# Prisma-Multimodal/ViT-Prisma

Hardware: NVIDIA H100
Metric: SAE training tokens/sec (TopK SAE, d_model=768, dict=768x32, k=32) (higher is better)
Workload: dtype fp32

## Files before the change

vit-prisma_b200/csrc/sae.cu:

```cuda
#include "common.cuh"
#include "tc_common.cuh"
#include "sae_optim.cuh"

template <int CHUNKS>
__global__ void __launch_bounds__(256) k_sae_prep(const float* __restrict__ x, const float* __restrict__ b_dec, float* __restrict__ sae_in,
                                                  float* __restrict__ sae_in_lo, __half* __restrict__ sae_in16, float* __restrict__ mu_out,
                                                  float* __restrict__ std_out, int rows, int d, int norm_mode, float eps) {
  pb_pdl();
  const int lane = threadIdx.x & 31;
  const int row = blockIdx.x * (blockDim.x >> 5) + (threadIdx.x >> 5);
  if (row >= rows) return;
  const int nvec = d >> 2;
  const float* xr = x + (int64_t)row * d;
  float v[CHUNKS][4];
  float sum = 0.f;
#pragma unroll
  for (int i = 0; i < CHUNKS; ++i) {
    const int c4 = i * 32 + lane;
    if (c4 < nvec) { ld4(xr + 4 * c4, v[i]); sum += (v[i][0] + v[i][1]) + (v[i][2] + v[i][3]); }
    else v[i][0] = v[i][1] = v[i][2] = v[i][3] = 0.f;
  }
  float mu = 0.f, inv = 1.f, sd = 1.f;
  if (norm_mode == 1) {
    mu = warp_sum(sum) / (float)d;
// ... 277 lines not shown
      if (p < F) c.x = cnt[p];
      if (p + 1 < F) c.y = cnt[p + 1];
      if (p + 2 < F) c.z = cnt[p + 2];
    }
    v[i] = (int)c.x; v[i + 1] = (int)c.y; v[i + 2] = (int)c.z; v[i + 3] = (int)c.w;
  }
  int run = 0;
#pragma unroll
  for (int i = 0; i < PER; ++i) { const int x = v[i]; v[i] = run; run += x; }
  int x = run;
#pragma unroll
  for (int o = 1; o < 32; o <<= 1) {
    const int y = __shfl_up_sync(0xffffffffu, x, o);
    if (lane >= o) x += y;
  }
  if (lane == 31) wtot[warp] = x;
  __syncthreads();
  if (warp == 0) {
    int w = wtot[lane];
#pragma unroll
    for (int o = 1; o < 32; o <<= 1) {
      const int y = __shfl_up_sync(0xffffffffu, w, o);
      if (lane >= o) w += y;
    }
    wtot[lane] = w;
  }
  __syncthreads();
  const int excl = (warp ? wtot[warp - 1] : 0) + x - run;
#pragma unroll
  for (int i = 0; i < PER; i += 4) {
    const int p = base + i;
    const int4 o4 = make_int4(excl + v[i], excl + v[i + 1], excl + v[i + 2], excl + v[i + 3]);
    if (p + 3 < F) {
      *reinterpret_cast<int4*>(off + p) = o4;
      *reinterpret_cast<int4*>(cursor + p) = o4;
    } else {
      const int o[4] = {o4.x, o4.y, o4.z, o4.w};
      for (int j = 0; j < 4; ++j)
        if (p + j < F) { off[p + j] = o[j]; cursor[p + j] = o[j]; }
    }
  }
  if (t == 1023) off[F] = wtot[31];
}
__global__ void __launch_bounds__(256) k_csc_fill(const int* __restrict__ idx, int* __restrict__ cursor, int* __restrict__ entries, int64_t n) {
  pb_pdl();
  for (int64_t e = (int64_t)blockIdx.x * blockDim.x + threadIdx.x; e < n; e += (int64_t)gridDim.x * blockDim.x) {
    const int f = idx[e];
    const int pos = atomicAdd(cursor + f, 1);
    entries[pos] = (int)e;
  }
}

constexpr int SAE_LONG_LIST = 32;
constexpr int SAE_LONG_CHUNK = 32;
struct SaeWorkHeader { int n_chunks, n_long, next_f, pad; };
constexpr int SAE_CLAIM = 4;

template <int CHUNKS>
__global__ void __launch_bounds__(256) k_sae_grads(const int* __restrict__ off, int* __restrict__ entries, const float* __restrict__ val,
                                                   const float* __restrict__ dval, const float* __restrict__ g, const float* __restrict__ sae_in,
                                                   const float* __restrict__ W_encT, float* __restrict__ gW_dec, float* __restrict__ gW_encT,
                                                   float* __restrict__ gb_enc, float* __restrict__ gbdec2, float* __restrict__ fired,
                                                   SaeScalars* __restrict__ sc, int F, int d, int k, SaeWorkHeader* __restrict__ work,
                                                   int* __restrict__ work_feats, int* __restrict__ work_chunks) {
  pb_pdl();
  extern __shared__ __align__(16) float sm_bd[];
  const int lane = threadIdx.x & 31, warp = threadIdx.x >> 5, nw = blockDim.x >> 5;
  const int nvec = d >> 2;
  for (int c = threadIdx.x; c < d; c += blockDim.x) sm_bd[c] = 0.f;
  __syncthreads();
  float nsq = 0.f;
  float bd[CHUNKS][4];
#pragma unroll
  for (int i = 0; i < CHUNKS; ++i) bd[i][0] = bd[i][1] = bd[i][2] = bd[i][3] = 0.f;
  for (;;) {
    int fbase = 0;
    if (lane == 0) fbase = atomicAdd(&work->next_f, SAE_CLAIM);
    fbase = __shfl_sync(0xffffffffu, fbase, 0);
    if (fbase >= F) break;
   for (int f = fbase; f < min(F, fbase + SAE_CLAIM); ++f) {
    const int e0 = off[f], e1 = off[f + 1];
    const int len = e1 - e0;
    if (len > SAE_LONG_LIST) {
#pragma unroll
      for (int i = 0; i < CHUNKS; ++i) {
        const int c4 = i * 32 + lane;
        if (c4 < nvec) {
          const float z4[4] = {0.f, 0.f, 0.f, 0.f};
          st4(gW_dec + (int64_t)f * d + 4 * c4, z4);
          st4(gW_encT + (int64_t)f * d + 4 * c4, z4);
        }
      }
      const int nchunks = (len + SAE_LONG_CHUNK - 1) / SAE_LONG_CHUNK;
      int base = 0, lslot = 0;
      if (lane == 0) {
        gb_enc[f] = 0.f;
        fired[f] = 0.f;
        base = atomicAdd(&work->n_chunks, nchunks);
        lslot = atomicAdd(&work->n_long, 1);
        work_feats[lslot] = f;
      }
      base = __shfl_sync(0xffffffffu, base, 0);
      for (int c = lane; c < nchunks; c += 32) {
        work_chunks[2 * (base + c)] = f;
        work_chunks[2 * (base + c) + 1] = e0 + c * SAE_LONG_CHUNK;
      }
      continue;
    }
    int my_b = 0;
    float my_a = 0.f, my_dp = 0.f;
    {
      const int mine = lane < len ? entries[e0 + lane] : 0x7fffffff;
      int rank = 0;
#pragma unroll
      for (int j = 0; j < 32; ++j) rank += __shfl_sync(0xffffffffu, mine, j) < mine ? 1 : 0;
      int src = 0;
#pragma unroll
      for (int j = 0; j < 32; ++j) src = (__shfl_sync(0xffffffffu, rank, j) == lane && j < len) ? j : src;
      const int sorted = __shfl_sync(0xffffffffu, mine, src);
      if (lane < len) {
        my_b = sorted / k;
        my_a = fmaxf(val[sorted], 0.f);
        my_dp = dval[sorted];
      }
    }
    float ad[CHUNKS][4], ae[CHUNKS][4];
#pragma unroll
    for (int i = 0; i < CHUNKS; ++i) ad[i][0] = ad[i][1] = ad[i][2] = ad[i][3] = ae[i][0] = ae[i][1] = ae[i][2] = ae[i][3] = 0.f;
    float gbe = 0.f;
    const float npos = (float)__popc(__ballot_sync(0xffffffffu, my_a > 0.f));
#pragma unroll 2
    for (int j = 0; j < len; ++j) {
      const float a = __shfl_sync(0xffffffffu, my_a, j), dp = __shfl_sync(0xffffffffu, my_dp, j);
      const int b = __shfl_sync(0xffffffffu, my_b, j);
      gbe += dp;
      const float* gr = g + (int64_t)b * d;
      const float* sr = sae_in + (int64_t)b * d;
#pragma unroll
      for (int i = 0; i < CHUNKS; ++i) {
        const int c4 = i * 32 + lane;
        if (c4 < nvec) {
          float gv[4], sv[4];
          ld4(gr + 4 * c4, gv);
          ld4(sr + 4 * c4, sv);
#pragma unroll
          for (int q = 0; q < 4; ++q) { ad[i][q] = fmaf(a, gv[q], ad[i][q]); ae[i][q] = fmaf(dp, sv[q], ae[i][q]); }
        }
      }
    }
#pragma unroll
    for (int i = 0; i < CHUNKS; ++i) {
      const int c4 = i * 32 + lane;
      if (c4 < nvec) {
        st4(gW_dec + (int64_t)f * d + 4 * c4, ad[i]);
        st4(gW_encT + (int64_t)f * d + 4 * c4, ae[i]);
#pragma unroll
        for (int q = 0; q < 4; ++q) nsq += ad[i][q] * ad[i][q] + ae[i][q] * ae[i][q];
        if (gbe != 0.f) {
          float w[4];
          ld4(W_encT + (int64_t)f * d + 4 * c4, w);
#pragma unroll
          for (int q = 0; q < 4; ++q) bd[i][q] = fmaf(gbe, w[q], bd[i][q]);
        }
      }
    }
    if (lane == 0) {
      gb_enc[f] = gbe;
      fired[f] = npos;
      nsq += gbe * gbe;
    }
   }
  }
#pragma unroll
  for (int i = 0; i < CHUNKS; ++i) {
    const int c4 = i * 32 + lane;
    if (c4 < nvec) {
#pragma unroll
      for (int q = 0; q < 4; ++q)
        if (bd[i][q] != 0.f) atomicAdd(&sm_bd[4 * c4 + q], bd[i][q]);
    }
  }
  nsq = warp_sum(nsq);
  __shared__ float red[8];
  if (lane == 0) red[warp] = nsq;
  __syncthreads();
  if (threadIdx.x == 0) {
    float a = 0.f;
    for (int i = 0; i < nw; ++i) a += red[i];
    atomicAdd(&sc->gnorm_sq, a);
  }
  for (int c = threadIdx.x; c < d; c += blockDim.x)
    if (sm_bd[c] != 0.f) atomicAdd(gbdec2 + c, sm_bd[c]);
}

template <int CHUNKS>
__global__ void __launch_bounds__(256) k_sae_grads_long(const int* __restrict__ off, const int* __restrict__ entries, const float* __restrict__ val,
                                                        const float* __restrict__ dval, const float* __restrict__ g,
                                                        const float* __restrict__ sae_in, const float* __restrict__ W_encT,
                                                        float* __restrict__ gW_dec, float* __restrict__ gW_encT, float* __restrict__ gb_enc,
                                                        float* __restrict__ gbdec2, float* __restrict__ fired, int d, int k,
                                                        const SaeWorkHeader* __restrict__ work, const int* __restrict__ work_chunks) {
  pb_pdl();
  extern __shared__ __align__(16) float sm_bd[];
  const int lane = threadIdx.x & 31, warp = threadIdx.x >> 5, nw = blockDim.x >> 5;
  const int nvec = d >> 2;
  const int n_items = work->n_chunks;
  if (n_items == 0) return;
  for (int c = threadIdx.x; c < d; c += blockDim.x) sm_bd[c] = 0.f;
  __syncthreads();
  float bd[CHUNKS][4];
#pragma unroll
  for (int i = 0; i < CHUNKS; ++i) bd[i][0] = bd[i][1] = bd[i][2] = bd[i][3] = 0.f;
  for (int item = blockIdx.x * nw + warp; item < n_items; item += gridDim.x * nw) {
    const int f = work_chunks[2 * item], p0 = work_chunks[2 * item + 1];
    const int p1 = min(off[f + 1], p0 + SAE_LONG_CHUNK);
    float ad[CHUNKS][4], ae[CHUNKS][4];
#pragma unroll
    for (int i = 0; i < CHUNKS; ++i) ad[i][0] = ad[i][1] = ad[i][2] = ad[i][3] = ae[i][0] = ae[i][1] = ae[i][2] = ae[i][3] = 0.f;
    const int n = p1 - p0;
    int my_b = 0;
    float my_a = 0.f, my_dp = 0.f;
    if (lane < n) {
      const int e = entries[p0 + lane];
      my_b = e / k;
      my_a = fmaxf(val[e], 0.f);
      my_dp = dval[e];
    }
    float gbe = 0.f;
    const float npos = (float)__popc(__ballot_sync(0xffffffffu, my_a > 0.f));
#pragma unroll 2
    for (int j = 0; j < n; ++j) {
      const float a = __shfl_sync(0xffffffffu, my_a, j), dp = __shfl_sync(0xffffffffu, my_dp, j);
      const int b = __shfl_sync(0xffffffffu, my_b, j);
      gbe += dp;
      const float* gr = g + (int64_t)b * d;
      const float* sr = sae_in + (int64_t)b * d;
#pragma unroll
      for (int i = 0; i < CHUNKS; ++i) {
        const int c4 = i * 32 + lane;
        if (c4 < nvec) {
          float gv[4], sv[4];
          ld4(gr + 4 * c4, gv);
          ld4(sr + 4 * c4, sv);
#pragma unroll
          for (int q = 0; q < 4; ++q) { ad[i][q] = fmaf(a, gv[q], ad[i][q]); ae[i][q] = fmaf(dp, sv[q], ae[i][q]); }
        }
      }
    }
#pragma unroll
    for (int i = 0; i < CHUNKS; ++i) {
      const int c4 = i * 32 + lane;
      if (c4 < nvec) {
        atomicAdd(reinterpret_cast<float4*>(gW_dec + (int64_t)f * d + 4 * c4), make_float4(ad[i][0], ad[i][1], ad[i][2], ad[i][3]));
        atomicAdd(reinterpret_cast<float4*>(gW_encT + (int64_t)f * d + 4 * c4), make_float4(ae[i][0], ae[i][1], ae[i][2], ae[i][3]));
        if (gbe != 0.f) {
          float w[4];
          ld4(W_encT + (int64_t)f * d + 4 * c4, w);
#pragma unroll
          for (int q = 0; q < 4; ++q) bd[i][q] = fmaf(gbe, w[q], bd[i][q]);
        }
      }
    }
    if (lane == 0) {
      atomicAdd(gb_enc + f, gbe);
      atomicAdd(fired + f, npos);
    }
  }
#pragma unroll
  for (int i = 0; i < CHUNKS; ++i) {
    const int c4 = i * 32 + lane;
    if (c4 < nvec) {
#pragma unroll
      for (int q = 0; q < 4; ++q)
        if (bd[i][q] != 0.f) atomicAdd(&sm_bd[4 * c4 + q], bd[i][q]);
    }
  }
  __syncthreads();
  for (int c = threadIdx.x; c < d; c += blockDim.x)
    if (sm_bd[c] != 0.f) atomicAdd(gbdec2 + c, sm_bd[c]);
}

__global__ void __launch_bounds__(256) k_sae_norm_long(const float* __restrict__ gW_dec, const float* __restrict__ gW_encT,
                                                       const float* __restrict__ gb_enc, SaeScalars* __restrict__ sc, int d,
                                                       const SaeWorkHeader* work, const int* __restrict__ work_feats) {
  pb_pdl();
  const int lane = threadIdx.x & 31, warp = threadIdx.x >> 5, nw = blockDim.x >> 5;
  const int n = *reinterpret_cast<const volatile int*>(&work->n_long);
  float nsq = 0.f;
  for (int li = blockIdx.x * nw + warp; li < n; li += gridDim.x * nw) {
    const int f = work_feats[li];
    for (int c = lane; c < d; c += 32) {
      const float a = gW_dec[(int64_t)f * d + c], b = gW_encT[(int64_t)f * d + c];
      nsq += a * a + b * b;
    }
    if (lane == 0) nsq += gb_enc[f] * gb_enc[f];
  }
  nsq = warp_sum(nsq);
  if (lane == 0 && nsq != 0.f) atomicAdd(&sc->gnorm_sq, nsq);
}

__global__ void k_sae_gbdec(const float* __restrict__ gcol, const float* __restrict__ gbdec2, float* __restrict__ gb_dec, int d) {
  const int c = blockIdx.x * blockDim.x + threadIdx.x;
  if (c < d) gb_dec[c] = gcol[c] - gbdec2[c];
}

__global__ void __launch_bounds__(256) k_sae_finalize(const float* __restrict__ gcol, const float* __restrict__ gbdec2, float* __restrict__ gb_dec,
                                                      SaeScalars* __restrict__ sc, int d, float max_norm, float inv_elems, float inv_rows) {
  pb_pdl();
  __shared__ float red[8];
  float s = 0.f;
  for (int c = threadIdx.x; c < d; c += blockDim.x) {
    const float v = gcol[c] - gbdec2[c];
    gb_dec[c] = v;
    s += v * v;
  }
  s = warp_sum(s);
  if ((threadIdx.x & 31) == 0) red[threadIdx.x >> 5] = s;
  __syncthreads();
  if (threadIdx.x == 0) {
    float t = sc->gnorm_sq;
    for (int i = 0; i < 8; ++i) t += red[i];
    sae_publish_scalars(sc, t, max_norm, inv_elems, inv_rows);
  }
}

struct AdamRowsOut {
  float *W_dec, *W_encT, *W_encT_lo;
  __half* W_encT16;
  int64_t base;
  __device__ __forceinline__ void dec(int c4, const float (&w)[4]) const { st4(W_dec + base + 4 * c4, w); }
  __device__ __forceinline__ void enc(int c4, const float (&p)[4], const float (&lo)[4], uint2 p16) const {
    st4(W_encT + base + 4 * c4, p);
    if (W_encT_lo) st4(W_encT_lo + base + 4 * c4, lo);
    if (W_encT16) *reinterpret_cast<uint2*>(W_encT16 + base + 4 * c4) = p16;
  }
};

__device__ __forceinline__ void atomic_max_norm(float* out, float best_sq) {
  if (best_sq > 0.f) atomicMax(reinterpret_cast<unsigned int*>(out), __float_as_uint(sqrtf(best_sq)));
}

template <int CHUNKS>
__global__ void __launch_bounds__(256) k_sae_adam_rows(float* __restrict__ W_dec, float* __restrict__ W_encT, float* __restrict__ W_encT_lo,
                                                       __half* __restrict__ W_encT16, float* __restrict__ enc16_lo_max,
                                                       float* __restrict__ b_enc, const float* __restrict__ gW_dec,
                                                       const float* __restrict__ gW_encT, const float* __restrict__ gb_enc,
                                                       float* __restrict__ m_dec, float* __restrict__ v_dec, float* __restrict__ m_enc,
                                                       float* __restrict__ v_enc, float* __restrict__ m_be, float* __restrict__ v_be,
                                                       const float* __restrict__ fired, float* __restrict__ since_fired,
                                                       float* __restrict__ act_freq, const SaeScalars* __restrict__ sc, AdamHyper h,
                                                       int F, int d, int renorm, float* __restrict__ enc_norm_max) {
// ... 299 lines not shown
}

extern "C" int pb_sae_step_reset(const PbSaeStep* s, int32_t* fb_count, pb_stream_t stream) {
  PB_CHECK_ARG(s && s->feat_count && s->scalars && s->gcol && s->gbdec2, "pb_sae_step_reset: missing pointers");
  PB_CHECK_ARG(!s->work || s->work_bytes >= (int64_t)sizeof(SaeWorkHeader), "pb_sae_step_reset: work buffer too small");
  const int n = s->F > s->d ? s->F : s->d;
  int grid = (n + 255) / 256;
  if (grid > pb_sm_count() * 2) grid = pb_sm_count() * 2;
  if (grid * 256 < s->d) grid = (s->d + 255) / 256;
  PB_LAUNCH_PDL(k_sae_step_reset, grid, 256, 0, (cudaStream_t)stream, s->feat_count, s->F, (float*)s->scalars, s->gcol, s->gbdec2, s->d, (int*)s->work, fb_count);
  return PB_OK;
}

extern "C" int pb_sae_decode(const PbSaeStep* s, pb_stream_t stream) {
  PB_CHECK_ARG(s && s->x && s->xsum && s->idx && s->val && s->W_dec && s->b_dec && s->scalars, "pb_sae_decode: missing pointers");
  PB_CHECK_ARG(!s->training || (s->g && s->dval), "pb_sae_decode: training needs g and dval buffers");
  if (s->rows == 0) return PB_OK;
  cudaStream_t st = (cudaStream_t)stream;
  const int d = s->d, ch = chunks_for(d);
  PB_DISPATCH_CHUNKS(ch, PB_LAUNCH_PDL(k_sae_decode<C_>, (s->rows + 7) / 8, 256, 0, st,
      s->x, s->xsum, s->mu, s->sd, s->idx, s->val, s->W_dec, s->b_dec, s->sae_out, s->g, s->dval, (SaeScalars*)s->scalars, s->rows, d, s->k,
      s->norm_mode, s->training, 1.f / (float)(s->global_rows > 0 ? s->global_rows : s->rows)));
  if (!s->training) {
    k_sae_fwd_scalars<<<1, 1, 0, st>>>((SaeScalars*)s->scalars, 1.f / ((float)s->rows * (float)d), 1.f / (float)s->rows);
    PB_LAUNCH_CHECK();
  }
  return PB_OK;
}

extern "C" int pb_sae_backward(const PbSaeStep* s, pb_stream_t stream) {
  PB_CHECK_ARG(s && s->idx && s->val && s->dval && s->g && s->sae_in && s->W_encT && s->feat_count && s->csc_off && s->csc_cursor &&
               s->csc_entries && s->gW_dec && s->gW_encT && s->gb_enc && s->gb_dec && s->gcol && s->gbdec2 && s->fired && s->scalars,
               "pb_sae_backward: missing pointers");
  if (s->rows == 0) return PB_OK;
  cudaStream_t st = (cudaStream_t)stream;
  const int d = s->d, F = s->F, ch = chunks_for(d);
  {
    const int per = ((F + 1023) / 1024 + 3) / 4 * 4;
    PB_CHECK_ARG(per <= 128, "pb_sae_backward: d_sae=%d too large for the offset scan (max 131072)", F);
    if (per <= 8) PB_LAUNCH_PDL(k_scan_counts<8>, 1, 1024, 0, st, s->feat_count, s->csc_off, s->csc_cursor, F);
    else if (per <= 24) PB_LAUNCH_PDL(k_scan_counts<24>, 1, 1024, 0, st, s->feat_count, s->csc_off, s->csc_cursor, F);
    else if (per <= 48) PB_LAUNCH_PDL(k_scan_counts<48>, 1, 1024, 0, st, s->feat_count, s->csc_off, s->csc_cursor, F);
    else if (per <= 64) PB_LAUNCH_PDL(k_scan_counts<64>, 1, 1024, 0, st, s->feat_count, s->csc_off, s->csc_cursor, F);
    else PB_LAUNCH_PDL(k_scan_counts<128>, 1, 1024, 0, st, s->feat_count, s->csc_off, s->csc_cursor, F);
  }
  const int64_t n = (int64_t)s->rows * s->k;
  PB_LAUNCH_PDL(k_csc_fill, pb_sm_count() * 4, 256, 0, st, (const int*)s->idx, s->csc_cursor, s->csc_entries, n);
  if (!s->pre_zeroed) {
    PB_CUDA(cudaMemsetAsync(s->gcol, 0, sizeof(float) * d, st));
    PB_CUDA(cudaMemsetAsync(s->gbdec2, 0, sizeof(float) * d, st));
  }
  const int rpc = 8;
  PB_LAUNCH_PDL(k_colsum, (s->rows + rpc - 1) / rpc, 256, 0, st, (const float*)s->g, s->gcol, s->rows, d, rpc);
  const int64_t cap = n / SAE_LONG_CHUNK + F + 1;
  const int64_t need = (int64_t)sizeof(SaeWorkHeader) + 4 * (int64_t)F + 8 * cap;
  PB_CHECK_ARG(s->work && s->work_bytes >= need, "pb_sae_backward: work buffer too small (%lld < %lld bytes)", (long long)s->work_bytes,
               (long long)need);
  SaeWorkHeader* wh = (SaeWorkHeader*)s->work;
  int* work_feats = (int*)(wh + 1);
  int* work_chunks = work_feats + F;
  if (!s->pre_zeroed) PB_CUDA(cudaMemsetAsync(wh, 0, sizeof(SaeWorkHeader), st));
  const int grid = persistent_grid(8, F);
  PB_DISPATCH_CHUNKS(ch, PB_LAUNCH_PDL(k_sae_grads<C_>, grid, 256, sizeof(float) * d, st, s->csc_off, s->csc_entries, s->val, s->dval, s->g, s->sae_in,
                                       s->W_encT, s->gW_dec, s->gW_encT, s->gb_enc, s->gbdec2, s->fired, (SaeScalars*)s->scalars, F, d, s->k, wh,
                                       work_feats, work_chunks));
  PB_DISPATCH_CHUNKS(ch, PB_LAUNCH_PDL(k_sae_grads_long<C_>, pb_sm_count() * 4, 256, sizeof(float) * d, st, s->csc_off, s->csc_entries, s->val, s->dval,
                                       s->g, s->sae_in, s->W_encT, s->gW_dec, s->gW_encT, s->gb_enc, s->gbdec2, s->fired, d, s->k, wh, work_chunks));
  if (!s->dist) {
    PB_LAUNCH_PDL(k_sae_norm_long, pb_sm_count(), 256, 0, st, s->gW_dec, s->gW_encT, s->gb_enc, (SaeScalars*)s->scalars, d, wh, work_feats);
  }
  if (s->dist) {
    k_sae_gbdec<<<(d + 255) / 256, 256, 0, st>>>(s->gcol, s->gbdec2, s->gb_dec, d);
    PB_LAUNCH_CHECK();
    return PB_OK;
  }
  PB_LAUNCH_PDL(k_sae_finalize, 1, 256, 0, st, s->gcol, s->gbdec2, s->gb_dec, (SaeScalars*)s->scalars, d, s->max_grad_norm,
                1.f / ((float)s->rows * (float)d), 1.f / (float)s->rows);
  return PB_OK;
}

extern "C" int pb_sae_adam(const PbSaeStep* s, pb_stream_t stream) {
  PB_CHECK_ARG(s && s->W_dec && s->W_encT && s->b_enc && s->b_dec && s->gW_dec && s->gW_encT && s->gb_enc && s->gb_dec && s->m_dec &&
               s->v_dec && s->m_enc && s->v_enc && s->m_be && s->v_be && s->m_bd && s->v_bd && s->fired && s->scalars,
               "pb_sae_adam: missing pointers");
  PB_CHECK_ARG(s->step >= 1, "pb_sae_adam: step counter starts at 1");
  cudaStream_t st = (cudaStream_t)stream;
  const int d = s->d, F = s->F, ch = chunks_for(d);
  const AdamHyper h = adam_hyper(s->lr, s->beta1, s->beta2, s->adam_eps, s->step);
  const int grid = persistent_grid(8, F);
  PB_CHECK_ARG(!s->W_encT16 == !s->enc16_lo_max, "pb_sae_adam: W_encT16 and enc16_lo_max go together");
  PB_CHECK_ARG(!s->W_encT16 || (d % 8 == 0 && ((uintptr_t)s->W_encT16 & 15) == 0), "pb_sae_adam: the fp16 copy of W_encT needs d %% 8 == 0");
  __half* const W16 = (__half*)s->W_encT16;
  if (s->enc_norm_max) PB_CUDA(cudaMemsetAsync(s->enc_norm_max, 0, 2 * sizeof(float), st));
  if (s->enc16_lo_max) PB_CUDA(cudaMemsetAsync(s->enc16_lo_max, 0, sizeof(float), st));
  if (!s->W_encT_lo && d >= 64) {
    const size_t stage = (size_t)8 * d * 4;
    int S = (int)((200 * 1024) / stage);
    if (S > 12) S = 12;
    if (S >= 3) {
      const size_t smem = 256 + (size_t)S * stage;
      int g2 = pb_sm_count();
      if (g2 > F) g2 = F;
      PB_DISPATCH_CHUNKS(ch, {
        auto kern = k_sae_adam_bulk<C_>;
        PB_CUDA(cudaFuncSetAttribute(kern, cudaFuncAttributeMaxDynamicSharedMemorySize, (int)smem));
        PB_LAUNCH_PDL(kern, g2, 32 * (1 + S), smem, st, s->W_dec, s->W_encT, s->b_enc, s->gW_dec, s->gW_encT, s->gb_enc, s->m_dec, s->v_dec,
                      s->m_enc, s->v_enc, s->m_be, s->v_be, s->fired, s->since_fired, s->act_freq, (const SaeScalars*)s->scalars, h, F, d,
                      s->renorm_decoder, s->enc_norm_max, S, s->b_dec, s->gb_dec, s->m_bd, s->v_bd, W16, s->enc16_lo_max);
      });
      return PB_OK;
    }
  }
  PB_DISPATCH_CHUNKS(ch, (k_sae_adam_rows<C_><<<grid, 256, 0, st>>>(s->W_dec, s->W_encT, s->W_encT_lo, W16, s->enc16_lo_max, s->b_enc, s->gW_dec,
                                                                     s->gW_encT, s->gb_enc,
                                                                     s->m_dec, s->v_dec, s->m_enc, s->v_enc, s->m_be, s->v_be, s->fired,
                                                                     s->since_fired, s->act_freq, (const SaeScalars*)s->scalars, h,
                                                                     F, d, s->renorm_decoder, s->enc_norm_max)));
  PB_LAUNCH_CHECK();
  k_sae_adam_vec<<<(d + 255) / 256, 256, 0, st>>>(s->b_dec, s->gb_dec, s->m_bd, s->v_bd, (const SaeScalars*)s->scalars, h, d);
  PB_LAUNCH_CHECK();
  return PB_OK;
}
// ... 63 lines not shown
```

vit-prisma_b200/vit_prisma/b200/sae_engine.py:

```python
from __future__ import annotations

import ctypes as C
from typing import Optional

import torch

from . import _lib as L
from .ops import _need_cuda, _stream, cast as _cast


def ops_cast_f32(x: torch.Tensor) -> torch.Tensor:
    return _cast(x.contiguous(), torch.float32)

vp, i32, i64, f32 = C.c_void_p, C.c_int32, C.c_int64, C.c_float


class PbSaeStep(C.Structure):
    _fields_ = (
        [(n, i32) for n in ("rows", "d", "F", "k", "norm_mode", "training", "step", "renorm_decoder")]
        + [(n, f32) for n in ("lr", "beta1", "beta2", "adam_eps", "max_grad_norm")]
        + [(n, vp) for n in (
            "x", "W_encT", "W_encT_lo", "W_dec", "b_enc", "b_dec",
            "sae_in", "mu", "sd", "xsum", "idx", "val", "feat_count", "sae_out", "g", "dval",
            "csc_off", "csc_cursor", "csc_entries", "gW_dec", "gW_encT", "gb_enc", "gb_dec", "gcol", "gbdec2",
# ... 116 lines not shown
            encoder = "fused" if (fused_ok and gemm_impl == L.GEMM_AUTO) else "dense"
        if encoder == "fused" and not fused_ok:
            raise L.PrismaB200Error(f"fused encoder->TopK needs d_in % 4 == 0, d_sae % 128 == 0, k <= 48 (d={self.d} F={self.F} k={self.k})")
        self.cand_operands = ("f16" if f16_ok else "tf32") if encoder == "fused" else None
        import os
        self.encoder, self.c_keep = encoder, int(os.environ.get("PRISMA_SAE_C_KEEP", c_keep))
        self.m_cand = int(os.environ.get("PRISMA_SAE_M_CAND", 0)) or (int(m_cand) if m_cand else self.k + 8)
        self.enc_norm_max = z(2)
        self.fb_count = z(2, dt=torch.int32)
        self.W_encT_lo = torch.empty_like(W_encT) if encoder == "dense" else None
        f16 = self.cand_operands == "f16"
        self.W_encT16 = torch.empty(self.F, self.d, dtype=torch.float16, device=dev) if f16 else None
        self.enc16_lo_max = z(1) if f16 else None
        self.refresh_lo()
        self.m_dec, self.v_dec, self.m_enc, self.v_enc = z(self.F, self.d), z(self.F, self.d), z(self.F, self.d), z(self.F, self.d)
        self.m_be, self.v_be, self.m_bd, self.v_bd = z(self.F), z(self.F), z(self.d), z(self.d)
        self.gW_dec, self.gW_encT = torch.empty(self.F, self.d, device=dev), torch.empty(self.F, self.d, device=dev)
        self.gb_enc, self.gb_dec = z(self.F), z(self.d)
        self.gcol, self.gbdec2, self.xsum = z(self.d), z(self.d), z(self.d)
        self.feat_count, self.fired = z(self.F), z(self.F)
        self.csc_off, self.csc_cursor = z(self.F + 1, dt=torch.int32), z(self.F, dt=torch.int32)
        self.scalars = z(8)
        self.step_count = 0
        self._rows = -1

    def refresh_lo(self) -> None:
        if self.W_encT_lo is not None:
            from . import ops
            self.W_encT_lo.copy_(ops.split_tf32(self.W_encT))
        L.check(L.get_lib().pb_rownorm_max(self.W_encT.data_ptr(), self.F, self.d, self.enc_norm_max.data_ptr(), _stream()), "pb_rownorm_max")
        if self.W_encT16 is not None:
            L.check(L.get_lib().pb_f16_copy(self.W_encT.data_ptr(), self.F, self.d, self.W_encT16.data_ptr(), self.enc16_lo_max.data_ptr(),
                                            _stream()), "pb_f16_copy")

    def _ensure_rows(self, rows: int) -> None:
        if rows == self._rows:
            return
        dev, d, F, k = self.W_dec.device, self.d, self.F, self.k
        e = lambda *s, dt=torch.float32: torch.empty(*s, dtype=dt, device=dev)
        self.sae_in, self.g, self.sae_out = e(rows, d), e(rows, d), e(rows, d)
        self.mu, self.sd = e(rows), e(rows)
        if self.encoder == "fused":
            cb, sb = i64(0), i64(0)
            L.check(L.get_lib().pb_sae_fused_workspace(rows, F, self.c_keep, C.byref(cb), C.byref(sb)), "pb_sae_fused_workspace")
            self.cand = e(max(cb.value // 4, 4), dt=torch.int32)
            self.fb_rows = e(max(rows, 1), dt=torch.int32)
            self.fb_scratch = e(min(64, max(sb.value // (4 * F), 1)) * F)
            self.sae_in_lo = self.hidden_pre = None
            self.sae_in16 = e(rows, d, dt=torch.float16) if self.cand_operands == "f16" else None
        else:
            self.sae_in_lo, self.hidden_pre = e(rows, d), e(rows, F)
        self.idx, self.val, self.dval = e(rows, k, dt=torch.int32), e(rows, k), e(rows, k)
        self.csc_entries = e(rows * k, dt=torch.int32)
        self.work = e(8 + 4 * F + 8 * (rows * k // 32 + F + 1) + 64, dt=torch.uint8)
        nseg = (F + TOPK_SEG - 1) // TOPK_SEG
        self.topk_scratch = e(max(rows * nseg * k * 8, 16), dt=torch.uint8) if F > TOPK_SEG else None
        self._rows = rows

    def _desc(self, x: torch.Tensor, training: bool, lr: float = 0.0, since_fired=None, act_freq=None, want_out=True) -> PbSaeStep:
        s = PbSaeStep()
        s.rows, s.d, s.F, s.k = x.shape[0], self.d, self.F, self.k
        s.norm_mode, s.training, s.step, s.renorm_decoder = self.norm_mode, int(training), max(self.step_count, 1), 1
        s.lr, s.beta1, s.beta2, s.adam_eps, s.max_grad_norm = lr, self.betas[0], self.betas[1], self.adam_eps, self.max_grad_norm
        p = lambda t: None if t is None else t.data_ptr()
        s.x = p(x)
        s.W_encT, s.W_encT_lo, s.W_dec, s.b_enc, s.b_dec = p(self.W_encT), p(self.W_encT_lo), p(self.W_dec), p(self.b_enc), p(self.b_dec)
        s.sae_in, s.mu, s.sd, s.xsum = p(self.sae_in), p(self.mu), p(self.sd), p(self.xsum)
        s.idx, s.val, s.feat_count = p(self.idx), p(self.val), p(self.feat_count)
        s.sae_out, s.g, s.dval = (p(self.sae_out) if want_out else None), p(self.g), p(self.dval)
        s.csc_off, s.csc_cursor, s.csc_entries = p(self.csc_off), p(self.csc_cursor), p(self.csc_entries)
        s.gW_dec, s.gW_encT, s.gb_enc, s.gb_dec = p(self.gW_dec), p(self.gW_encT), p(self.gb_enc), p(self.gb_dec)
        s.gcol, s.gbdec2, s.fired, s.scalars = p(self.gcol), p(self.gbdec2), p(self.fired), p(self.scalars)
        s.m_dec, s.v_dec, s.m_enc, s.v_enc = p(self.m_dec), p(self.v_dec), p(self.m_enc), p(self.v_enc)
        s.m_be, s.v_be, s.m_bd, s.v_bd = p(self.m_be), p(self.v_be), p(self.m_bd), p(self.v_bd)
        s.since_fired, s.act_freq = p(since_fired), p(act_freq)
        s.work, s.work_bytes = p(self.work), self.work.numel()
        s.enc_norm_max = p(self.enc_norm_max)
        s.W_encT16, s.enc16_lo_max = p(self.W_encT16), p(self.enc16_lo_max)
        return s

    def _enc_desc(self, rows: int, phases: int = 0) -> PbSaeEncode:
        e = PbSaeEncode()
        e.rows, e.d, e.F, e.k, e.c_keep, e.m_cand, e.phases, e.err_coef = rows, self.d, self.F, self.k, self.c_keep, self.m_cand, phases, 0.0
        e.sae_in, e.W_encT, e.b_enc, e.enc_norm_max = self.sae_in.data_ptr(), self.W_encT.data_ptr(), self.b_enc.data_ptr(), self.enc_norm_max.data_ptr()
        e.cand, e.cand_bytes = self.cand.data_ptr(), self.cand.numel() * 4
        e.idx, e.val, e.feat_count = self.idx.data_ptr(), self.val.data_ptr(), self.feat_count.data_ptr()
        e.fb_count, e.fb_rows = self.fb_count.data_ptr(), self.fb_rows.data_ptr()
        e.fb_scratch, e.fb_scratch_bytes = self.fb_scratch.data_ptr(), self.fb_scratch.numel() * 4
        if self.cand_operands == "f16":
            e.sae_in16, e.W_encT16, e.enc16_lo_max = self.sae_in16.data_ptr(), self.W_encT16.data_ptr(), self.enc16_lo_max.data_ptr()
        return e

    def _encoder_gemm(self, rows: int) -> None:
        lib, st = L.get_lib(), _stream()
        use_tc = self.gemm_impl != L.GEMM_SIMT
        g = L.PbGemm()
        g.M, g.N, g.K, g.dtype, g.impl = rows, self.F, self.d, L.PB_F32, self.gemm_impl
        g.A, g.lda, g.B, g.ldb = self.sae_in.data_ptr(), self.d, self.W_encT.data_ptr(), self.d
        if use_tc:
            g.A_lo, g.B_lo = self.sae_in_lo.data_ptr(), self.W_encT_lo.data_ptr()
        g.bias, g.out0, g.ld0 = self.b_enc.data_ptr(), self.hidden_pre.data_ptr(), self.F
        L.check(lib.pb_gemm(C.byref(g), st), "pb_gemm(encoder)")

    def encode_topk(self, x: torch.Tensor, pre_zeroed: bool = False) -> None:
        lib, st = L.get_lib(), _stream()
        rows = x.shape[0]
        self._ensure_rows(rows)
# ... 54 lines not shown
        return int(self.fb_count[0].item()) if self.encoder == "fused" else 0

    def rescored_per_row(self, rows: int) -> float:
        fb, tot = self.fb_count.tolist()
        return tot / max(rows - fb, 1)

    def _optimizer_stages(self, s: PbSaeStep, x: torch.Tensor, lr: float, since_fired, act_freq):
        lib, st = L.get_lib(), _stream()
        kernel = "k_sae_adam_rows" if self.W_encT_lo is not None or self.d < 64 else "k_sae_adam_bulk"
        f16_copy = 2 * self.d * self.F if self.W_encT16 is not None else 0
        return [("adam (clip + decoder-parallel-gradient removal + Adam + row renorm)", lambda: L.check(lib.pb_sae_adam(C.byref(s), st)),
                 dict(bytes=60 * self.d * self.F + f16_copy, ncu=kernel))]

    def _clip_and_adam(self, x: torch.Tensor, lr: float, since_fired, act_freq, grads, extra) -> None:
        lib, st = L.get_lib(), _stream()
        self.scalars[1:2].zero_()
        acc = self.scalars[1:].data_ptr()
        for t in grads:
            L.check(lib.pb_sumsq(t.data_ptr(), t.numel(), acc, st), "pb_sumsq")
        L.check(lib.pb_sae_clip_finish(self.scalars.data_ptr(), self.max_grad_norm, x.shape[0], self.d, st), "pb_sae_clip_finish")
        s = self._desc(x, training=True, lr=lr, since_fired=since_fired, act_freq=act_freq, want_out=False)
        L.check(lib.pb_sae_adam(C.byref(s), st), "pb_sae_adam")
        for p, g, m, v in extra:
            L.check(lib.pb_adam_vec(p.data_ptr(), g.data_ptr(), m.data_ptr(), v.data_ptr(), p.numel(), self.scalars.data_ptr(), lr, self.betas[0],
                                    self.betas[1], self.adam_eps, self.step_count, st), "pb_adam_vec")

    @torch.no_grad()
    def time_stages(self, x: torch.Tensor, lr: float, since_fired=None, act_freq=None, reps: int = 5) -> dict:
        lib, st = L.get_lib(), _stream()
        x = ops_cast_f32(x)
        rows = x.shape[0]
        out = {}

        def timed(name, fn, **info):
            torch.cuda.synchronize()
            a, b = torch.cuda.Event(enable_timing=True), torch.cuda.Event(enable_timing=True)
            a.record()
            for _ in range(reps):
                fn()
            b.record()
            torch.cuda.synchronize()
            out[name] = dict(ms=a.elapsed_time(b) / reps, **info)

        for name, fn, info in self._encode_stages(x):
            timed(name, fn, **info)
        self.encode_topk(x)
        self.scalars.zero_()
        self.step_count += 1
        s = self._desc(x, training=True, lr=float(lr), since_fired=since_fired, act_freq=act_freq, want_out=False)
        self._prepare_timed_step(s, x)
        timed("decode (sparse decode + loss + d_hidden)", lambda: L.check(lib.pb_sae_decode(C.byref(s), st)),
              bytes=(12 * rows * self.d + 8 * rows * self.k), ncu=r"k_sae_decode")
        timed("backward (csc build + per-feature gradients + norm)", lambda: (self.scalars.zero_(), L.check(lib.pb_sae_backward(C.byref(s), st))),
              bytes=8 * self.d * self.F, ncu=r"k_sae_grads<")
        for name, fn, info in self._optimizer_stages(s, x, float(lr), since_fired, act_freq):
            timed(name, fn, **info)
        return out

    def _prepare_timed_step(self, s: PbSaeStep, x: torch.Tensor) -> None:
        pass

    def _encode_stages(self, x: torch.Tensor):
        rows = x.shape[0]
        if self.encoder == "fused":
            lib, st = L.get_lib(), _stream()
            self.encode_topk(x)
            flops = 2.0 * rows * self.d * self.F
            nkeys = (self.F // 128) * self.c_keep
            op, es = ("fp16", 2) if self.cand_operands == "f16" else ("tf32", 4)
            return [(f"encode + topk, fused (prep + {op} candidate GEMM + select / exact re-score + exact path)", lambda: self.encode_topk(x),
                     dict(flops=flops, passes=1)),
                    (f"candidate GEMM alone (one {op} pass, top-c-per-segment epilogue)",
                     lambda: L.check(lib.pb_sae_encode_topk_fused(C.byref(self._enc_desc(rows, 1)), st)),
                     dict(flops=flops, passes=1, bytes=es * self.d * self.F + es * rows * self.d + 4 * rows * nkeys, ncu=r"k_enc_cand")),
                    ("select + exact re-score alone", lambda: L.check(lib.pb_sae_encode_topk_fused(C.byref(self._enc_desc(rows, 2)), st)),
                     dict(bytes=4 * rows * nkeys + 4 * rows * self.d + 8 * rows * self.k, ncu=r"k_cand_select"))]
        return [("encode + topk (prep + encoder GEMM 3xTF32 + exact topk)", lambda: self.encode_topk(x),
                 dict(flops=2.0 * rows * self.d * self.F, passes=3, ncu=r"k_gemm_tc<float")),
                ("encoder GEMM alone (hidden_pre = sae_in @ W_enc + b_enc)", lambda: self._encoder_gemm(rows),
                 dict(flops=2.0 * rows * self.d * self.F, passes=3, bytes=8 * self.d * self.F + 8 * rows * self.d + 4 * rows * self.F))]

    def dense_feature_acts(self) -> torch.Tensor:
        rows = self.idx.shape[0]
        dense = torch.empty(rows, self.F, device=self.W_dec.device)
        L.check(L.get_lib().pb_sae_scatter_acts(self.idx.data_ptr(), self.val.data_ptr(), dense.data_ptr(), rows, self.k, self.F, 1,
                                                _stream()), "pb_sae_scatter_acts")
        return dense

    def scalars_dict(self) -> dict:
        vals = self.scalars.tolist()
        return dict(zip(SCALAR_NAMES, vals))

    def algorithmic_bytes(self, rows: int) -> int:
        return 80 * self.d * self.F + 8 * rows * self.d
```

Baseline: 3.038 million.

## Replace chunked long-feature gradient path with token-sorted pack and column-sliced smem kernel

Features with many firing tokens are no longer split into 32-entry chunks that accumulate into the weight gradients with float4 atomics. A new pack kernel sorts each long feature's entries by token using a bitmap and prefix sums, and writes packed token, activation and d-value arrays. It also computes gb_enc, fired and the bias norm term. A column-sliced kernel then stages 8-column slices of g and sae_in for all rows in shared memory and lets each warp compute the full gradient for one feature over that slice, writing the result directly and folding in the norm, which removes the separate norm kernel. This trades global gather traffic and atomics for a large shared-memory footprint, row chunking with binary searches when rows exceed the smem capacity, and an added cap on rows from the bitmap.

```diff
diff --git a/vit-prisma_b200/csrc/sae.cu b/vit-prisma_b200/csrc/sae.cu
--- a/vit-prisma_b200/csrc/sae.cu
+++ b/vit-prisma_b200/csrc/sae.cu
@@ -353,9 +353,12 @@
 }
 
 constexpr int SAE_LONG_LIST = 32;
-constexpr int SAE_LONG_CHUNK = 32;
-struct SaeWorkHeader { int n_chunks, n_long, next_f, pad; };
+struct SaeWorkHeader { int next_f, n_long, pad[2]; };
 constexpr int SAE_CLAIM = 4;
+constexpr int SAE_SLICE = 8;
+constexpr int SAE_SLICE_THREADS = 1024;
+constexpr int SAE_SLICE_PARTS = 2;
+constexpr int SAE_SLICE_SMEM = 192 * 1024;
 
 template <int CHUNKS>
 __global__ void __launch_bounds__(256) k_sae_grads(const int* __restrict__ off, int* __restrict__ entries, const float* __restrict__ val,
@@ -363,7 +366,7 @@
                                                    const float* __restrict__ W_encT, float* __restrict__ gW_dec, float* __restrict__ gW_encT,
                                                    float* __restrict__ gb_enc, float* __restrict__ gbdec2, float* __restrict__ fired,
                                                    SaeScalars* __restrict__ sc, int F, int d, int k, SaeWorkHeader* __restrict__ work,
-                                                   int* __restrict__ work_feats, int* __restrict__ work_chunks) {
+                                                   int* __restrict__ work_feats) {
   pb_pdl();
   extern __shared__ __align__(16) float sm_bd[];
   const int lane = threadIdx.x & 31, warp = threadIdx.x >> 5, nw = blockDim.x >> 5;
@@ -383,29 +386,7 @@
     const int e0 = off[f], e1 = off[f + 1];
     const int len = e1 - e0;
     if (len > SAE_LONG_LIST) {
-#pragma unroll
-      for (int i = 0; i < CHUNKS; ++i) {
-        const int c4 = i * 32 + lane;
-        if (c4 < nvec) {
-          const float z4[4] = {0.f, 0.f, 0.f, 0.f};
-          st4(gW_dec + (int64_t)f * d + 4 * c4, z4);
-          st4(gW_encT + (int64_t)f * d + 4 * c4, z4);
-        }
-      }
-      const int nchunks = (len + SAE_LONG_CHUNK - 1) / SAE_LONG_CHUNK;
-      int base = 0, lslot = 0;
-      if (lane == 0) {
-        gb_enc[f] = 0.f;
-        fired[f] = 0.f;
-        base = atomicAdd(&work->n_chunks, nchunks);
-        lslot = atomicAdd(&work->n_long, 1);
-        work_feats[lslot] = f;
-      }
-      base = __shfl_sync(0xffffffffu, base, 0);
-      for (int c = lane; c < nchunks; c += 32) {
-        work_chunks[2 * (base + c)] = f;
-        work_chunks[2 * (base + c) + 1] = e0 + c * SAE_LONG_CHUNK;
-      }
+      if (lane == 0) work_feats[atomicAdd(&work->n_long, 1)] = f;
       continue;
     }
     int my_b = 0;
@@ -494,110 +475,184 @@
     if (sm_bd[c] != 0.f) atomicAdd(gbdec2 + c, sm_bd[c]);
 }
 
-template <int CHUNKS>
-__global__ void __launch_bounds__(256) k_sae_grads_long(const int* __restrict__ off, const int* __restrict__ entries, const float* __restrict__ val,
-                                                        const float* __restrict__ dval, const float* __restrict__ g,
-                                                        const float* __restrict__ sae_in, const float* __restrict__ W_encT,
-                                                        float* __restrict__ gW_dec, float* __restrict__ gW_encT, float* __restrict__ gb_enc,
-                                                        float* __restrict__ gbdec2, float* __restrict__ fired, int d, int k,
-                                                        const SaeWorkHeader* __restrict__ work, const int* __restrict__ work_chunks) {
+__global__ void __launch_bounds__(256) k_sae_pack_long(const int* __restrict__ off, const int* __restrict__ entries, const float* __restrict__ val,
+                                                       const float* __restrict__ dval, int* __restrict__ ptok, float* __restrict__ pa,
+                                                       float* __restrict__ pd, float* __restrict__ gb_enc, float* __restrict__ fired,
+                                                       SaeScalars* __restrict__ sc, int rows, int k, const SaeWorkHeader* work,
+                                                       const int* __restrict__ work_feats) {
   pb_pdl();
-  extern __shared__ __align__(16) float sm_bd[];
-  const int lane = threadIdx.x & 31, warp = threadIdx.x >> 5, nw = blockDim.x >> 5;
-  const int nvec = d >> 2;
-  const int n_items = work->n_chunks;
-  if (n_items == 0) return;
-  for (int c = threadIdx.x; c < d; c += blockDim.x) sm_bd[c] = 0.f;
+  extern __shared__ unsigned int pk_smem[];
+  const int nw = (rows + 31) >> 5;
+  unsigned int* bm = pk_smem;
+  unsigned int* pre = pk_smem + nw;
+  __shared__ int wtot[8];
+  __shared__ float red[2][8];
+  const int t = threadIdx.x, lane = t & 31, warp = t >> 5;
+  const int n_long = *reinterpret_cast<const volatile int*>(&work->n_long);
+  const int per = (nw + 255) / 256;
+  for (int li = blockIdx.x; li < n_long; li += gridDim.x) {
+    const int f = work_feats[li];
+    const int e0 = off[f], e1 = off[f + 1], len = e1 - e0;
+    for (int w = t; w < nw; w += 256) bm[w] = 0u;
+    __syncthreads();
+    for (int i = e0 + t; i < e1; i += 256) {
+      const int b = entries[i] / k;
+      atomicOr(&bm[b >> 5], 1u << (b & 31));
+    }
+    __syncthreads();
+    int run = 0;
+    for (int w = t * per; w < min(nw, (t + 1) * per); ++w) run += __popc(bm[w]);
+    int x = run;
+#pragma unroll
+    for (int o = 1; o < 32; o <<= 1) {
+      const int y = __shfl_up_sync(0xffffffffu, x, o);
+      if (lane >= o) x += y;
+    }
+    if (lane == 31) wtot[warp] = x;
+    __syncthreads();
+    int base = x - run;
+    for (int w = 0; w < warp; ++w) base += wtot[w];
+    for (int w = t * per; w < min(nw, (t + 1) * per); ++w) { pre[w] = base; base += __popc(bm[w]); }
+    __syncthreads();
+    float npos = 0.f;
+    for (int i = e0 + t; i < e1; i += 256) {
+      const int e = entries[i], b = e / k;
+      const int pos = e0 + pre[b >> 5] + __popc(bm[b >> 5] & ((1u << (b & 31)) - 1u));
+      const float a = fmaxf(val[e], 0.f);
+      ptok[pos] = b;
+      pa[pos] = a;
+      pd[pos] = dval[e];
+      npos += a > 0.f ? 1.f : 0.f;
+    }
+    __syncthreads();
+    const int q = (len + 255) / 256;
+    float gbe = 0.f;
+    for (int i = e0 + t * q; i < min(e1, e0 + (t + 1) * q); ++i) gbe += pd[i];
+    gbe = warp_sum(gbe);
+    npos = warp_sum(npos);
+    if (lane == 0) { red[0][warp] = gbe; red[1][warp] = npos; }
+    __syncthreads();
+    if (t == 0) {
+      float g = 0.f, n = 0.f;
+      for (int w = 0; w < 8; ++w) { g += red[0][w]; n += red[1][w]; }
+      gb_enc[f] = g;
+      fired[f] = n;
+      atomicAdd(&sc->gnorm_sq, g * g);
+    }
+    __syncthreads();
+  }
+}
+
+__device__ __forceinline__ int lower_bound_tok(const int* __restrict__ tok, int lo, int hi, int b) {
+  while (lo < hi) {
+    const int mid = (lo + hi) >> 1;
+    if (tok[mid] < b) lo = mid + 1;
+    else hi = mid;
+  }
+  return lo;
+}
+
+__global__ void __launch_bounds__(SAE_SLICE_THREADS) k_sae_grads_slices(const int* __restrict__ off, const int* __restrict__ ptok,
+                                                                        const float* __restrict__ pa, const float* __restrict__ pd,
+                                                                        const float* __restrict__ g, const float* __restrict__ sae_in,
+                                                                        const float* __restrict__ W_encT, const float* __restrict__ gb_enc,
+                                                                        float* __restrict__ gW_dec, float* __restrict__ gW_encT,
+                                                                        float* __restrict__ gbdec2, SaeScalars* __restrict__ sc, int rows,
+                                                                        int d, int chunk_rows, const SaeWorkHeader* work,
+                                                                        const int* __restrict__ work_feats) {
+  pb_pdl();
+  extern __shared__ __align__(16) float sl[];
+  constexpr int NW = SAE_SLICE_THREADS / 32;
+  __shared__ float red_n[NW], red_b[NW][SAE_SLICE];
+  __shared__ int next_list;
+  const int t = threadIdx.x, lane = t & 31, warp = t >> 5;
+  const int enc = blockIdx.x & 1, part = (blockIdx.x >> 1) % SAE_SLICE_PARTS, c0 = (blockIdx.x >> 1) / SAE_SLICE_PARTS * SAE_SLICE;
+  const int col = c0 + lane;
+  const bool writer = lane < SAE_SLICE && col < d;
+  const float* __restrict__ X = enc ? sae_in : g;
+  const float* __restrict__ coef = enc ? pd : pa;
+  float* __restrict__ out = enc ? gW_encT : gW_dec;
+  const int n_long = *reinterpret_cast<const volatile int*>(&work->n_long);
+  const int l0 = (int)((int64_t)n_long * part / SAE_SLICE_PARTS), l1 = (int)((int64_t)n_long * (part + 1) / SAE_SLICE_PARTS);
+  float nsq = 0.f, bd = 0.f;
+  for (int r0 = 0; r0 < rows; r0 += chunk_rows) {
+    const int nr = min(chunk_rows, rows - r0);
+    const bool first = r0 == 0, last = r0 + nr == rows;
+    __syncthreads();
+    if (t == 0) next_list = l0;
+    for (int i0 = t; i0 < 2 * nr; i0 += 8 * SAE_SLICE_THREADS) {
+      float4 v[8];
+#pragma unroll
+      for (int u = 0; u < 8; ++u) {
+        const int i = i0 + u * SAE_SLICE_THREADS, cc = c0 + 4 * (i & 1);
+        v[u] = make_float4(0.f, 0.f, 0.f, 0.f);
+        if (i < 2 * nr && cc < d) v[u] = *reinterpret_cast<const float4*>(X + (int64_t)(r0 + (i >> 1)) * d + cc);
+      }
+#pragma unroll
+      for (int u = 0; u < 8; ++u) {
+        const int i = i0 + u * SAE_SLICE_THREADS, r = i >> 1;
+        if (i < 2 * nr) *reinterpret_cast<float4*>(sl + r * SAE_SLICE + 4 * ((i & 1) ^ ((r >> 2) & 1))) = v[u];
+      }
+    }
+    __syncthreads();
+    for (;;) {
+      int li = 0;
+      if (lane == 0) li = atomicAdd(&next_list, 1);
+      li = __shfl_sync(0xffffffffu, li, 0);
+      if (li >= l1) break;
+      const int f = work_feats[li];
+      int p0 = off[f], p1 = off[f + 1];
+      if (!(first && last)) {
+        p0 = lower_bound_tok(ptok, p0, p1, r0);
+        p1 = lower_bound_tok(ptok, p0, p1, r0 + nr);
+      }
+      float acc[SAE_SLICE];
+#pragma unroll
+      for (int q = 0; q < SAE_SLICE; ++q) acc[q] = 0.f;
+#pragma unroll 4
+      for (int p = p0 + lane; p < p1; p += 32) {
+        const int r = ptok[p] - r0;
+        const float w = coef[p];
+        const int s = (r >> 2) & 1;
+        const float4 x0 = *reinterpret_cast<const float4*>(sl + r * SAE_SLICE + 4 * s);
+        const float4 x1 = *reinterpret_cast<const float4*>(sl + r * SAE_SLICE + 4 * (s ^ 1));
+        acc[0] = fmaf(w, x0.x, acc[0]); acc[1] = fmaf(w, x0.y, acc[1]); acc[2] = fmaf(w, x0.z, acc[2]); acc[3] = fmaf(w, x0.w, acc[3]);
+        acc[4] = fmaf(w, x1.x, acc[4]); acc[5] = fmaf(w, x1.y, acc[5]); acc[6] = fmaf(w, x1.z, acc[6]); acc[7] = fmaf(w, x1.w, acc[7]);
+      }
+      float mine = 0.f;
+#pragma unroll
+      for (int q = 0; q < SAE_SLICE; ++q) {
+        float v = acc[q];
+#pragma unroll
+        for (int o = 16; o > 0; o >>= 1) v += __shfl_xor_sync(0xffffffffu, v, o);
+        if (lane == q) mine = v;
+      }
+      if (writer) {
+        float* o = out + (int64_t)f * d + col;
+        const float v = first ? mine : *o + mine;
+        *o = v;
+        if (last) {
+          nsq += v * v;
+          const float gbe = enc ? gb_enc[f] : 0.f;
+          if (gbe != 0.f) bd = fmaf(gbe, W_encT[(int64_t)f * d + col], bd);
+        }
+      }
+    }
+  }
+  nsq = warp_sum(nsq);
+  if (lane == 0) red_n[warp] = nsq;
+  if (lane < SAE_SLICE) red_b[warp][lane] = bd;
   __syncthreads();
-  float bd[CHUNKS][4];
-#pragma unroll
-  for (int i = 0; i < CHUNKS; ++i) bd[i][0] = bd[i][1] = bd[i][2] = bd[i][3] = 0.f;
-  for (int item = blockIdx.x * nw + warp; item < n_items; item += gridDim.x * nw) {
-    const int f = work_chunks[2 * item], p0 = work_chunks[2 * item + 1];
-    const int p1 = min(off[f + 1], p0 + SAE_LONG_CHUNK);
-    float ad[CHUNKS][4], ae[CHUNKS][4];
-#pragma unroll
-    for (int i = 0; i < CHUNKS; ++i) ad[i][0] = ad[i][1] = ad[i][2] = ad[i][3] = ae[i][0] = ae[i][1] = ae[i][2] = ae[i][3] = 0.f;
-    const int n = p1 - p0;
-    int my_b = 0;
-    float my_a = 0.f, my_dp = 0.f;
-    if (lane < n) {
-      const int e = entries[p0 + lane];
-      my_b = e / k;
-      my_a = fmaxf(val[e], 0.f);
-      my_dp = dval[e];
-    }
-    float gbe = 0.f;
-    const float npos = (float)__popc(__ballot_sync(0xffffffffu, my_a > 0.f));
-#pragma unroll 2
-    for (int j = 0; j < n; ++j) {
-      const float a = __shfl_sync(0xffffffffu, my_a, j), dp = __shfl_sync(0xffffffffu, my_dp, j);
-      const int b = __shfl_sync(0xffffffffu, my_b, j);
-      gbe += dp;
-      const float* gr = g + (int64_t)b * d;
-      const float* sr = sae_in + (int64_t)b * d;
-#pragma unroll
-      for (int i = 0; i < CHUNKS; ++i) {
-        const int c4 = i * 32 + lane;
-        if (c4 < nvec) {
-          float gv[4], sv[4];
-          ld4(gr + 4 * c4, gv);
-          ld4(sr + 4 * c4, sv);
-#pragma unroll
-          for (int q = 0; q < 4; ++q) { ad[i][q] = fmaf(a, gv[q], ad[i][q]); ae[i][q] = fmaf(dp, sv[q], ae[i][q]); }
-        }
-      }
-    }
-#pragma unroll
-    for (int i = 0; i < CHUNKS; ++i) {
-      const int c4 = i * 32 + lane;
-      if (c4 < nvec) {
-        atomicAdd(reinterpret_cast<float4*>(gW_dec + (int64_t)f * d + 4 * c4), make_float4(ad[i][0], ad[i][1], ad[i][2], ad[i][3]));
-        atomicAdd(reinterpret_cast<float4*>(gW_encT + (int64_t)f * d + 4 * c4), make_float4(ae[i][0], ae[i][1], ae[i][2], ae[i][3]));
-        if (gbe != 0.f) {
-          float w[4];
-          ld4(W_encT + (int64_t)f * d + 4 * c4, w);
-#pragma unroll
-          for (int q = 0; q < 4; ++q) bd[i][q] = fmaf(gbe, w[q], bd[i][q]);
-        }
-      }
-    }
-    if (lane == 0) {
-      atomicAdd(gb_enc + f, gbe);
-      atomicAdd(fired + f, npos);
-    }
-  }
-#pragma unroll
-  for (int i = 0; i < CHUNKS; ++i) {
-    const int c4 = i * 32 + lane;
-    if (c4 < nvec) {
-#pragma unroll
-      for (int q = 0; q < 4; ++q)
-        if (bd[i][q] != 0.f) atomicAdd(&sm_bd[4 * c4 + q], bd[i][q]);
-    }
-  }
-  __syncthreads();
-  for (int c = threadIdx.x; c < d; c += blockDim.x)
-    if (sm_bd[c] != 0.f) atomicAdd(gbdec2 + c, sm_bd[c]);
-}
-
-__global__ void __launch_bounds__(256) k_sae_norm_long(const float* __restrict__ gW_dec, const float* __restrict__ gW_encT,
-                                                       const float* __restrict__ gb_enc, SaeScalars* __restrict__ sc, int d,
-                                                       const SaeWorkHeader* work, const int* __restrict__ work_feats) {
-  pb_pdl();
-  const int lane = threadIdx.x & 31, warp = threadIdx.x >> 5, nw = blockDim.x >> 5;
-  const int n = *reinterpret_cast<const volatile int*>(&work->n_long);
-  float nsq = 0.f;
-  for (int li = blockIdx.x * nw + warp; li < n; li += gridDim.x * nw) {
-    const int f = work_feats[li];
-    for (int c = lane; c < d; c += 32) {
-      const float a = gW_dec[(int64_t)f * d + c], b = gW_encT[(int64_t)f * d + c];
-      nsq += a * a + b * b;
-    }
-    if (lane == 0) nsq += gb_enc[f] * gb_enc[f];
-  }
-  nsq = warp_sum(nsq);
-  if (lane == 0 && nsq != 0.f) atomicAdd(&sc->gnorm_sq, nsq);
+  if (t == 0) {
+    float a = 0.f;
+    for (int w = 0; w < NW; ++w) a += red_n[w];
+    if (a != 0.f) atomicAdd(&sc->gnorm_sq, a);
+  }
+  if (enc && t < SAE_SLICE && c0 + t < d) {
+    float a = 0.f;
+    for (int w = 0; w < NW; ++w) a += red_b[w][t];
+    if (a != 0.f) atomicAdd(gbdec2 + c0 + t, a);
+  }
 }
 
 __global__ void k_sae_gbdec(const float* __restrict__ gcol, const float* __restrict__ gbdec2, float* __restrict__ gb_dec, int d) {
@@ -1003,22 +1058,34 @@
   }
   const int rpc = 8;
   PB_LAUNCH_PDL(k_colsum, (s->rows + rpc - 1) / rpc, 256, 0, st, (const float*)s->g, s->gcol, s->rows, d, rpc);
-  const int64_t cap = n / SAE_LONG_CHUNK + F + 1;
-  const int64_t need = (int64_t)sizeof(SaeWorkHeader) + 4 * (int64_t)F + 8 * cap;
+  const int64_t need = (int64_t)sizeof(SaeWorkHeader) + 4 * (int64_t)F + 12 * n;
   PB_CHECK_ARG(s->work && s->work_bytes >= need, "pb_sae_backward: work buffer too small (%lld < %lld bytes)", (long long)s->work_bytes,
                (long long)need);
+  const int nw = (s->rows + 31) / 32;
+  PB_CHECK_ARG(8 * (int64_t)nw <= SAE_SLICE_SMEM, "pb_sae_backward: rows=%d too many for the token bitmap", s->rows);
   SaeWorkHeader* wh = (SaeWorkHeader*)s->work;
   int* work_feats = (int*)(wh + 1);
-  int* work_chunks = work_feats + F;
+  int* ptok = work_feats + F;
+  float* pa = (float*)(ptok + n);
+  float* pd = pa + n;
   if (!s->pre_zeroed) PB_CUDA(cudaMemsetAsync(wh, 0, sizeof(SaeWorkHeader), st));
   const int grid = persistent_grid(8, F);
   PB_DISPATCH_CHUNKS(ch, PB_LAUNCH_PDL(k_sae_grads<C_>, grid, 256, sizeof(float) * d, st, s->csc_off, s->csc_entries, s->val, s->dval, s->g, s->sae_in,
                                        s->W_encT, s->gW_dec, s->gW_encT, s->gb_enc, s->gbdec2, s->fired, (SaeScalars*)s->scalars, F, d, s->k, wh,
-                                       work_feats, work_chunks));
-  PB_DISPATCH_CHUNKS(ch, PB_LAUNCH_PDL(k_sae_grads_long<C_>, pb_sm_count() * 4, 256, sizeof(float) * d, st, s->csc_off, s->csc_entries, s->val, s->dval,
-                                       s->g, s->sae_in, s->W_encT, s->gW_dec, s->gW_encT, s->gb_enc, s->gbdec2, s->fired, d, s->k, wh, work_chunks));
-  if (!s->dist) {
-    PB_LAUNCH_PDL(k_sae_norm_long, pb_sm_count(), 256, 0, st, s->gW_dec, s->gW_encT, s->gb_enc, (SaeScalars*)s->scalars, d, wh, work_feats);
+                                       work_feats));
+  {
+    const size_t smem = 8 * (size_t)nw;
+    if (smem > 48 * 1024) PB_CUDA(cudaFuncSetAttribute(k_sae_pack_long, cudaFuncAttributeMaxDynamicSharedMemorySize, (int)smem));
+    PB_LAUNCH_PDL(k_sae_pack_long, pb_sm_count() * 4, 256, smem, st, s->csc_off, s->csc_entries, s->val, s->dval, ptok, pa, pd, s->gb_enc, s->fired,
+                  (SaeScalars*)s->scalars, s->rows, s->k, wh, work_feats);
+  }
+  {
+    const int chunk_rows = s->rows < SAE_SLICE_SMEM / (SAE_SLICE * 4) ? s->rows : SAE_SLICE_SMEM / (SAE_SLICE * 4);
+    const size_t smem = (size_t)chunk_rows * SAE_SLICE * 4;
+    if (smem > 48 * 1024) PB_CUDA(cudaFuncSetAttribute(k_sae_grads_slices, cudaFuncAttributeMaxDynamicSharedMemorySize, (int)smem));
+    const int slices = (d + SAE_SLICE - 1) / SAE_SLICE;
+    PB_LAUNCH_PDL(k_sae_grads_slices, 2 * SAE_SLICE_PARTS * slices, SAE_SLICE_THREADS, smem, st, s->csc_off, ptok, pa, pd, s->g, s->sae_in, s->W_encT, s->gb_enc,
+                  s->gW_dec, s->gW_encT, s->gbdec2, (SaeScalars*)s->scalars, s->rows, d, chunk_rows, wh, work_feats);
   }
   if (s->dist) {
     k_sae_gbdec<<<(d + 255) / 256, 256, 0, st>>>(s->gcol, s->gbdec2, s->gb_dec, d);
diff --git a/vit-prisma_b200/vit_prisma/b200/sae_engine.py b/vit-prisma_b200/vit_prisma/b200/sae_engine.py
--- a/vit-prisma_b200/vit_prisma/b200/sae_engine.py
+++ b/vit-prisma_b200/vit_prisma/b200/sae_engine.py
@@ -192,7 +192,7 @@
             self.sae_in_lo, self.hidden_pre = e(rows, d), e(rows, F)
         self.idx, self.val, self.dval = e(rows, k, dt=torch.int32), e(rows, k), e(rows, k)
         self.csc_entries = e(rows * k, dt=torch.int32)
-        self.work = e(8 + 4 * F + 8 * (rows * k // 32 + F + 1) + 64, dt=torch.uint8)
+        self.work = e(16 + 4 * F + 12 * rows * k + 64, dt=torch.uint8)
         nseg = (F + TOPK_SEG - 1) // TOPK_SEG
         self.topk_scratch = e(max(rows * nseg * k * 8, 16), dt=torch.uint8) if F > TOPK_SEG else None
         self._rows = rows
@@ -353,7 +353,7 @@
         timed("decode (sparse decode + loss + d_hidden)", lambda: L.check(lib.pb_sae_decode(C.byref(s), st)),
               bytes=(12 * rows * self.d + 8 * rows * self.k), ncu=r"k_sae_decode")
         timed("backward (csc build + per-feature gradients + norm)", lambda: (self.scalars.zero_(), L.check(lib.pb_sae_backward(C.byref(s), st))),
-              bytes=8 * self.d * self.F, ncu=r"k_sae_grads<")
+              bytes=8 * self.d * self.F, ncu=r"k_sae_grads_slices")
         for name, fn, info in self._optimizer_stages(s, x, float(lr), since_fired, act_freq):
             timed(name, fn, **info)
         return out
```

Result: slower. 2.941 million, median of 6 (-3.2%).
